# markomih/SplatFields

Hardware: AMD Instinct MI355X
Metric: splats*px rasterized/sec (fwd+bwd) (higher is better)
Workload: dtype f32

## Files before the change

### include/splatraster.h

```cpp
#ifndef SPLATRASTER_H
#define SPLATRASTER_H

#include <stddef.h>

#ifdef __cplusplus
extern "C" {
#endif

#define SR_VERSION 4
#define SR_TILE 16

typedef struct SrView {
    int image_height;
    int image_width;
    float tanfovx;
    float tanfovy;
    float scale_modifier;
    int sh_degree;
    int sh_coeffs;
    int prefiltered;
    int debug;
    const float* viewmatrix;
    const float* projmatrix;
    const float* campos;
// ... 218 lines not shown
    int count, rank, capacity;
} SrResFieldJob;
int sr_resfield_compose(int n_jobs, const SrResFieldJob* jobs, const long long* frame, void* hip_stream);
size_t sr_resfield_backward_workspace(int n_jobs, const SrResFieldJob* jobs);
int sr_resfield_backward(int n_jobs, const SrResFieldJob* jobs, const long long* frame, void* workspace, size_t workspace_bytes,
                         void* hip_stream);

size_t sr_triplane_backward_workspace(int n_points, int channels, int height, int width);
int sr_triplane_forward(int n_points, int channels, int height, int width, const float* planes, float* planes_texel_major,
                        const float* points, float* out, void* hip_stream);
int sr_triplane_backward(int n_points, int channels, int height, int width, const float* planes_texel_major, const float* points,
                         const float* dL_dout, float* dL_dplanes, float* dL_dpoints, void* workspace, void* hip_stream);

int sr_debug_layout(int n_splats, int height, int width, long long instances, size_t* out4);

int sr_debug_backward_stats(unsigned long long* out16, int reset);

int sr_debug_counters(long long* out4, int reset);

int sr_debug_snapshot(const SrView* view, const SrSplats* splats, const float* dL_dcolor, const float* dL_ddepth,
                      const float* dL_dalpha, int backward);

#define SR_PROFILE_STAGES 7
int sr_profile_enable(int on);
int sr_profile_collect(double* ms_sum, long long* launches);
const char* sr_profile_stage_name(int stage);

#ifdef __cplusplus
}
#endif
#endif
// ... 1 lines not shown
```

### splatfields_amd/csrc/api.hip

```cpp
#include <cstdint>
#include <cstdio>
#include <cstdlib>
#include <cstring>
#include <atomic>
#include <chrono>
#include <thread>
#include <mutex>
#include <string>
#include <vector>
#include "kernels.h"

namespace {

thread_local std::string g_last_error;
thread_local long long g_last_longest = -1;

int fail(const std::string& msg) { g_last_error = msg; return 1; }

int check_hip(hipError_t e, const char* what) {
    if (e == hipSuccess) return 0;
    return fail(std::string(what) + ": " + hipGetErrorString(e));
}

#define SR_TRY(expr) do { if (int rc_ = (expr)) return rc_; } while (0)
// ... 205 lines not shown
    sr::SplatsK k;
    k.N = s->count; k.means3D = s->means3D; k.opacities = s->opacities; k.scales = s->scales;
    k.rotations = s->rotations; k.cov3D = s->cov3D_precomp; k.shs = s->shs; k.colors = s->colors_precomp;
    k.raw = s->raw_params; k.shs_rest = s->shs_rest;
    return k;
}

long long covered_by_hint(long long hint) { return hint <= 2048 ? 2048 : hint <= 4096 ? 4096 : hint <= 8192 ? 8192 : -1; }

struct Call {
    hipStream_t st = nullptr;
    sr::ViewK v; sr::SplatsK s;
    sr::Geom g; sr::Binning b; sr::Image im;
    void carve(const void* geom, void* binning, long long capacity, const void* image) {
        sr::carve_geom(const_cast<void*>(geom), s.N, v.H, v.W, &g);
        if (binning) sr::carve_binning(binning, capacity, &b);
        if (image) sr::carve_image(const_cast<void*>(image), v.H, v.W, &im);
    }
};

int open_call(Call& c, const CallContext& ctx, void* hip_stream) {
    SR_TRY(validate(ctx.view, ctx.splats));
    g_call = ctx;
    c.st = static_cast<hipStream_t>(hip_stream);
    c.v = make_view(ctx.view);
    c.s = make_splats(ctx.splats);
    return 0;
}

bool capacity_in_range(long long r) { return r >= 0 && r < (1ll << 32); }

}

extern "C" {

int sr_version(void) { return SR_VERSION; }
const char* sr_last_error(void) { return g_last_error.c_str(); }

size_t sr_geom_bytes(int n, int h, int w) { return sr::carve_geom(nullptr, n, h, w, nullptr); }
size_t sr_binning_bytes(long long r, int, int) { return sr::carve_binning(nullptr, r, nullptr); }
size_t sr_image_bytes(int h, int w) { return sr::carve_image(nullptr, h, w, nullptr); }
size_t sr_backward_scratch_bytes(long long r) {
    const size_t n = (size_t)(r > 0 ? r : 1);
    return sr::align_up(n * sr::kSlotFloats * sizeof(float), 256);
}

}

namespace {

int launch_stage1(const SrView* view, const sr::ViewK& v, const sr::SplatsK& s, const sr::Geom& g, int* radii, uint32_t* host_out,
                  uint32_t host_seq, hipStream_t st) {
    { StageTimer t_(0, st); sr::launch_preprocess(v, s, g, radii, st); }
    SR_TRY(after_launch(view, st, "preprocess"));
    { StageTimer t_(1, st); sr::launch_count_tiles(v, s.N, g, st); sr::launch_scan_small(v, s.N, g, host_out, host_seq, st); }
// ... 540 lines not shown
                         const float* dL_dout, float* dL_dplanes, float* dL_dpoints, void* workspace, void* hip_stream) {
    if (n_points < 0 || !planes_texel_major || (n_points > 0 && (!points || !dL_dout)) || (dL_dplanes && !workspace))
        return fail("bad arguments to sr_triplane_backward");
    const int rc = sr::launch_triplane_backward(n_points, channels, height, width, planes_texel_major, points, dL_dout, dL_dplanes, dL_dpoints,
                                                workspace, static_cast<hipStream_t>(hip_stream));
    if (rc == 1) return fail("sr_triplane_backward: channels must be a multiple of 4 in 4..128, height * width <= 2^30, 12 n_points < 2^32");
    if (rc) return fail("sr_triplane_backward: clearing the tile counters failed");
    return check_hip(hipGetLastError(), "triplane_backward");
}

int sr_debug_layout(int n, int h, int w, long long instances, size_t* out4) {
    if (!out4 || n < 0 || h <= 0 || w <= 0 || instances < 0) return fail("bad arguments to sr_debug_layout");
    sr::Geom g; sr::Binning b;
    char* const origin = reinterpret_cast<char*>(4096);
    sr::carve_geom(origin, n, h, w, &g);
    sr::carve_binning(origin, instances, &b);
    out4[0] = (size_t)(reinterpret_cast<char*>(g.tile_start) - origin);
    out4[1] = (size_t)(reinterpret_cast<char*>(b.sorted_id) - origin);
    out4[2] = (size_t)(reinterpret_cast<char*>(g.total) - origin);
    out4[3] = (size_t)(reinterpret_cast<char*>(g.offsets) - origin);
    return 0;
}

int sr_debug_backward_stats(unsigned long long* out8, int reset) {
    if (!out8) return fail("null pointer in sr_debug_backward_stats");
    if (hipDeviceSynchronize() != hipSuccess) return fail("sr_debug_backward_stats: device synchronisation failed");
    return sr::backward_stats(out8, reset) ? fail("sr_debug_backward_stats: counter copy failed") : 0;
}

int sr_debug_snapshot(const SrView* view, const SrSplats* splats, const float* dL_dcolor, const float* dL_ddepth, const float* dL_dalpha,
                      int backward) {
    if (!view || !splats) return fail("null view/splats");
    g_call = CallContext{view, splats, backward ? "snapshot_bw.dump" : "snapshot_fw.dump", dL_dcolor, dL_ddepth, dL_dalpha};
    dump_snapshot(backward ? "render_backward (test hook)" : "preprocess (test hook)");
    return 0;
}

int sr_profile_enable(int on) { g_prof_on = on != 0; return 0; }

int sr_profile_collect(double* ms_sum, long long* launches) {
    std::lock_guard<std::mutex> lock(g_prof_mutex);
    std::vector<ProfRec> open;
// ... 17 lines not shown
```

### splatfields_amd/csrc/blend_bwd.hip

```cpp
#include "kernels.h"

namespace sr {

namespace {

constexpr int kBucket = 16;
constexpr int kBlkEntries = 32;
constexpr int kBlocks = 8;
#ifndef SR_BWD_CAP
#define SR_BWD_CAP 752
#endif
#ifndef SR_BWD_CAP_DEPTH
#define SR_BWD_CAP_DEPTH 624
#endif
template <bool HAS_D> struct SlotCap { static constexpr int kCap = HAS_D ? SR_BWD_CAP_DEPTH : SR_BWD_CAP; };
constexpr int kCapSlack = 16;
static_assert(SR_BWD_CAP >= 256 && SR_BWD_CAP_DEPTH >= 256, "one quad's entries of a chunk must always fit");
#ifndef SR_BWD_WAVES_PER_SIMD
#define SR_BWD_WAVES_PER_SIMD 4
#endif

typedef float f32x4 __attribute__((ext_vector_type(4)));

#ifdef SR_BWD_STATS
__device__ unsigned long long g_bwd_stats[16];
#define SR_STAT_ADD(i, x) atomicAdd(&g_bwd_stats[i], (unsigned long long)(x))
#define SR_PHASE(i) do { const long long now_ = clock64(); ph_[i] += now_ - t_; t_ = now_; } while (0)
#else
#define SR_STAT_ADD(i, x) do {} while (0)
#define SR_PHASE(i) do {} while (0)
#endif

constexpr int kShr1 = 0x111, kShr2 = 0x112, kShr4 = 0x114, kShr8 = 0x118;

template <int CTRL> __device__ __forceinline__ float dpp_f(float old, float src) {
    return __int_as_float(__builtin_amdgcn_update_dpp(__float_as_int(old), __float_as_int(src), CTRL, 0xf, 0xf, false));
}
template <int CTRL> __device__ __forceinline__ uint32_t dpp_u(uint32_t old, uint32_t src) {
    return (uint32_t)__builtin_amdgcn_update_dpp((int)old, (int)src, CTRL, 0xf, 0xf, false);
}
// ... 63 lines not shown
    const float4 r3 = rec[3];
    e.rect_xy = __float_as_uint(r3.x); e.rect_w = __float_as_uint(r3.y); e.first_rel = __float_as_uint(r3.z);
    e.inst = g.block_offsets[id >> 8];
    e.ef = make_float2(0.f, 0.f);
    e.qm = qms[pc];
    return e;
}
__device__ __forceinline__ void finish_entry(BwdEntry& e, uint32_t tx, uint32_t ty) {
    float E0, F0, ps;
    exponent_terms(e.c.x, e.c.y, e.r1, (float)(tx * kTile), (float)(ty * kTile), E0, F0, ps);
    e.ef = make_float2(E0, F0);
    e.r1.y = ps;
    e.inst += e.first_rel + (ty - (e.rect_xy >> 16)) * e.rect_w + (tx - (e.rect_xy & 0xffffu));
}

template <bool HAS_D> struct SlotFmt { static constexpr int kF = HAS_D ? 12 : 10; };

struct SlotIn { float E0, F0, p, ps, q, nlo, r, g, b, depth; int pos; };

template <bool HAS_D>
__device__ __forceinline__ void slot_put_record(float* sl, const BwdEntry& e) {
    if constexpr (HAS_D) {
        float4* d = reinterpret_cast<float4*>(sl);
        d[0] = make_float4(e.ef.x, e.ef.y, __int_as_float(e.pos), e.r1.x);
        d[1] = make_float4(e.r1.y, e.r1.z, e.r1.w, e.r2.x);
        d[2] = make_float4(e.r2.y, e.r2.z, e.r2.w, 0.f);
    } else {
        float2* d = reinterpret_cast<float2*>(sl);
        d[0] = make_float2(e.ef.x, e.ef.y);
        d[1] = make_float2(__int_as_float(e.pos), e.r1.x);
        d[2] = make_float2(e.r1.y, e.r1.z);
        d[3] = make_float2(e.r1.w, e.r2.x);
        d[4] = make_float2(e.r2.y, e.r2.z);
    }
}
template <bool HAS_D>
__device__ __forceinline__ SlotIn slot_get_record(const float* sl) {
    SlotIn r;
    if constexpr (HAS_D) {
        const float4* d = reinterpret_cast<const float4*>(sl);
        const float4 a = d[0], b = d[1], c = d[2];
        r.E0 = a.x; r.F0 = a.y; r.pos = __float_as_int(a.z); r.p = a.w;
        r.ps = b.x; r.q = b.y; r.nlo = b.z; r.r = b.w;
        r.g = c.x; r.b = c.y; r.depth = c.z;
    } else {
        const float2* d = reinterpret_cast<const float2*>(sl);
        const float2 a = d[0], b = d[1], c = d[2], e = d[3], f = d[4];
        r.E0 = a.x; r.F0 = a.y; r.pos = __float_as_int(b.x); r.p = b.y;
        r.ps = c.x; r.q = c.y; r.nlo = e.x; r.r = e.y;
        r.g = f.x; r.b = f.y; r.depth = 0.f;
    }
    return r;
}
__device__ __forceinline__ void slot_mask_invalid(SlotIn& r, bool valid) {
    r.nlo = valid ? r.nlo : __builtin_inff();
    r.r = valid ? r.r : 0.f; r.g = valid ? r.g : 0.f; r.b = valid ? r.b : 0.f; r.depth = valid ? r.depth : 0.f;
}
struct BucketSums { float w0, w1, w2; };
__device__ __forceinline__ void slot_put_sums(float* sl, int row, const BucketSums d) {
    const int o64 = row == 0 ? 0 : row == 1 ? 6 : row == 2 ? 4 : 8;
    *reinterpret_cast<float2*>(sl + o64) = row == 2 ? make_float2(d.w1, d.w2) : make_float2(d.w0, d.w1);
    if ((row & 1) == 0) sl[row == 0 ? 2 : 3] = row == 0 ? d.w2 : d.w0;
}
template <bool HAS_D>
__device__ __forceinline__ void slot_get_sums(const float* sl, float4& a, float4& b, float2& c) {
    if constexpr (HAS_D) {
        const float4* d = reinterpret_cast<const float4*>(sl);
        const float4 x = d[0], y = d[1], z = d[2];
        a = make_float4(x.x, x.w, y.z, z.x); b = make_float4(x.y, y.x, y.w, z.y); c = make_float2(x.z, y.y);
    } else {
        const float2* d = reinterpret_cast<const float2*>(sl);
        const float2 x0 = d[0], x1 = d[1], x2 = d[2], x3 = d[3], x4 = d[4];
        a = make_float4(x0.x, x1.y, x3.x, x4.x); b = make_float4(x0.y, x2.x, x3.y, x4.y); c = make_float2(x1.x, x2.y);
    }
}

__constant__ float kColumn[3][16] = {
    {0.f, 1.f, 2.f, 3.f, 4.f, 5.f, 6.f, 7.f, 8.f, 9.f, 10.f, 11.f, 12.f, 13.f, 14.f, 15.f},
    {-7.5f, -6.5f, -5.5f, -4.5f, -3.5f, -2.5f, -1.5f, -0.5f, 0.5f, 1.5f, 2.5f, 3.5f, 4.5f, 5.5f, 6.5f, 7.5f},
    {56.25f, 42.25f, 30.25f, 20.25f, 12.25f, 6.25f, 2.25f, 0.25f, 0.25f, 2.25f, 6.25f, 12.25f, 20.25f, 30.25f, 42.25f, 56.25f}};

struct QuadCtx {
    float gR[4], gG[4], gB[4], gD[4], gA[4];
    int last[4];
    float Y;
    float Xa[4], Xc[4], Xc2[4];
};

#define SR_DPP_MUL4(ctrl) \
// ... 69 lines not shown
    const float Yc = c.Y - 7.5f;
    const float mY = Yc * a0, mXY = Yc * a1, mYY = Yc * mY;
    BucketSums r;
    r.w0 = swap16_sum(swap32_sum(a0, a1), swap32_sum(mY, a2));
    r.w1 = swap16_sum(swap32_sum(mXY, mYY), swap32_sum(br, bg));
    const float zz = swap32_sum(bb, bd);
    r.w2 = swap16_sum(zz, zz);
    (void)lane;
    return r;
}

template <bool HAS_D>
__global__ void __launch_bounds__(kBlock, SR_BWD_WAVES_PER_SIMD)
k_render_backward_quads(const ViewK v, const Geom g, const Binning b, const Image im, const float* __restrict__ dL_dcolor,
                       const float* __restrict__ dL_ddepth, const float* __restrict__ dL_dalpha, float* __restrict__ slots) {
    constexpr int kF = SlotFmt<HAS_D>::kF;
    constexpr int kCap = SlotCap<HAS_D>::kCap;
    __shared__ __attribute__((aligned(16))) float s_slot[(kCap + kCapSlack) * kF];
    __shared__ float4 s_pixA[256];
    __shared__ float4 s_pixB[256];
    __shared__ uint32_t s_mask[2][16][kBlocks];
    __shared__ uint16_t s_bb[2][16][kBlocks];
    __shared__ uint32_t s_qlen[2][16], s_qbase[2][16];
    __shared__ uint32_t s_ticket[2];

    const int tile = (int)g.tile_order[blockIdx.x];
    const int tx = tile % v.gx, ty = tile / v.gx;
    const int wave = wave_id(), lane = lane_id();
    const uint32_t start = g.tile_start[tile];
    const float tx0f = (float)(tx * kTile), ty0f = (float)(ty * kTile);
#ifdef SR_BWD_STATS
    long long ph_[8] = {0, 0, 0, 0, 0, 0, 0, 0}, t_ = clock64();
#endif
// ... 1 lines not shown
    const int tid = (int)threadIdx.x;
    const uint32_t* ids = b.sorted_id + start;

    uint32_t qlast[16];
    {
        const uint32_t* ql = g.tile_qlast + 16 * (size_t)tile;
#pragma unroll
        for (int q = 0; q < 16; ++q) qlast[q] = ql[q];
    }
    uint32_t bmax_u = 0u, qlast_min = 0xffffffffu;
#pragma unroll
    for (int q = 0; q < 16; ++q) { bmax_u = max(bmax_u, qlast[q]); qlast_min = min(qlast_min, qlast[q]); }
    const int bmax = __builtin_amdgcn_readfirstlane((int)bmax_u);
    qlast_min = (uint32_t)__builtin_amdgcn_readfirstlane((int)qlast_min);

    constexpr int kChunk = kBlocks * kBlkEntries;
    static_assert(kChunk == kBlock, "one list entry per thread");
    if (bmax == 0) return;
    int hi = bmax;
    const uint32_t* qms = b.qmask + start;
    const uint32_t id_first = ids[max(hi - 1 - tid, 0)];
    uint32_t id_next = ids[max(hi - kChunk - 1 - tid, 0)];
    BwdEntry cur = load_entry(g, id_first, qms, hi - 1 - tid);

    {
        const int lx = threadIdx.x & 15, ly = threadIdx.x >> 4;
        const int px = tx * kTile + lx, py = ty * kTile + ly;
        const bool inside = px < v.W && py < v.H;
        const size_t hw = (size_t)v.H * v.W, pix = (size_t)py * v.W + px;
        uint32_t my_last = 0;
        float T_final = 0.f, gR = 0.f, gG = 0.f, gB = 0.f, gD = 0.f, gA = 0.f;
        if (inside) {
            my_last = im.n_contrib[pix];
            T_final = im.final_T[pix];
            gR = dL_dcolor[pix]; gG = dL_dcolor[hw + pix]; gB = dL_dcolor[2 * hw + pix];
            if (HAS_D) gD = dL_ddepth[pix];
            if (dL_dalpha) gA = dL_dalpha[pix];
        }
// ... 2 lines not shown
        s_pixB[threadIdx.x] = make_float4(gA, __uint_as_float(my_last), T_final, T_final * bg_dot);
        if (threadIdx.x < 2) s_ticket[threadIdx.x] = 0u;
    }

    const int k = lane >> 4, nl = lane & 15;
    const uint32_t lt_mask = (1u << (lane & 31)) - 1u;
    const int myblk = (int)threadIdx.x >> 5;

    float4* slot4 = reinterpret_cast<float4*>(slots);
    const float4 zero4 = make_float4(0.f, 0.f, 0.f, 0.f);

    int par = 0;
    SR_PHASE(0);

    while (hi > 0) {
        uint32_t qm = 0u;
        if (cur.pos >= 0) {
            qm = cur.qm & 0xffffu;
            if ((uint32_t)cur.pos >= qlast_min) {
#pragma unroll
                for (int q = 0; q < 16; ++q) if ((uint32_t)cur.pos >= qlast[q]) qm &= ~(1u << q);
            }
        }
        {
            uint32_t mlo = 0u, mhi = 0u;
#pragma unroll
            for (int q = 0; q < 16; ++q) {
                const uint64_t bal = __builtin_amdgcn_ballot_w64(((qm >> q) & 1u) != 0u);
                asm("s_nop 3\n\tv_writelane_b32 %0, %2, %4\n\tv_writelane_b32 %1, %3, %4"
                    : "+v"(mlo), "+v"(mhi) : "s"((uint32_t)bal), "s"((uint32_t)(bal >> 32)), "n"(q));
// ... 22 lines not shown
                for (int qq = 0; qq < 16; ++qq) {
                    const uint32_t pq = (uint32_t)__builtin_amdgcn_readlane((int)len, qq);
                    if (run + pq > (uint32_t)kCap) { pass_starts |= 1u << qq; run = 0u; }
                    my_base = q == qq ? run : my_base;
                    run += pq;
                }
            }
            if (lane < 16) {
                s_qlen[par][q] = len; s_qbase[par][q] = my_base;
#pragma unroll
                for (int blk = 0; blk < kBlocks; ++blk) s_bb[par][q][blk] = (uint16_t)(my_base + first_of[blk]);
            }
            if (threadIdx.x == 0) s_ticket[par ^ 1] = 0u;
#ifdef SR_BWD_STATS
            { const uint32_t pairs = row_allsum_u32(len);
              if (threadIdx.x == 0) { SR_STAT_ADD(0, min(hi, kChunk)); SR_STAT_ADD(1, pairs); SR_STAT_ADD(5, 1); } }
#endif
            __builtin_amdgcn_fence(__ATOMIC_RELEASE, "wavefront");
            __builtin_amdgcn_wave_barrier();
            __builtin_amdgcn_fence(__ATOMIC_ACQUIRE, "wavefront");
        }
        float4 s0 = zero4, s1 = zero4;
        float2 s2 = make_float2(0.f, 0.f);
        pass_starts = (uint32_t)__builtin_amdgcn_readfirstlane((int)pass_starts) | 0x10000u;
        uint32_t last_pmask = 0u;
        auto combine = [&](uint32_t pmask) {
            if (cur.pos >= 0) {
                uint32_t m = qm & pmask;
                while (m) {
                    const int q = __builtin_ctz(m);
                    m &= m - 1u;
                    const uint32_t slot = (uint32_t)s_bb[par][q][myblk] + (uint32_t)__popc(s_mask[par][q][myblk] & lt_mask);
                    float4 a, cc; float2 d;
                    slot_get_sums<HAS_D>(s_slot + kF * slot, a, cc, d);
                    s0.x += a.x; s0.y += a.y; s0.z += a.z; s0.w += a.w;
                    s1.x += cc.x; s1.y += cc.y; s1.z += cc.z; s1.w += cc.w;
                    s2.x += d.x; if (HAS_D) s2.y += d.y;
                }
            }
        };
#pragma unroll 1
        for (int q_lo = 0; q_lo < 16;) {
            const int q_hi = __builtin_ctz(pass_starts & ~((2u << q_lo) - 1u));
            const uint32_t pmask = ((1u << q_hi) - 1u) & ~((1u << q_lo) - 1u);
            if (q_lo == 0) finish_entry(cur, (uint32_t)tx, (uint32_t)ty);
            {
                uint32_t m = qm & pmask;
                while (m) {
                    const int q = __builtin_ctz(m);
                    m &= m - 1u;
                    const uint32_t slot = (uint32_t)s_bb[par][q][myblk] + (uint32_t)__popc(s_mask[par][q][myblk] & lt_mask);
                    slot_put_record<HAS_D>(s_slot + kF * slot, cur);
                }
            }
            if (threadIdx.x == 0) s_ticket[par] = (uint32_t)q_lo;
            SR_PHASE(3);
            lds_barrier();
            SR_PHASE(4);
            uint32_t ticket = 0u;
            if (lane == 0) ticket = atomicAdd(&s_ticket[par], 1u);
#pragma unroll 1
            for (;;) {
                const int q = __builtin_amdgcn_readfirstlane((int)ticket);
                if (q >= q_hi) break;
                if (lane == 0) ticket = atomicAdd(&s_ticket[par], 1u);
                const int qy = q >> 2, qx = q & 3;
                const int len = __builtin_amdgcn_readfirstlane((int)s_qlen[par][q]);
// ... 2 lines not shown
                const int prow = (4 * qy + k) * 16 + 4 * qx;
                QuadCtx c;
                float ST[4], SB[4];
                c.Y = (float)(4 * qy + k);
#pragma unroll
                for (int t = 0; t < 4; ++t) {
                    c.Xa[t] = kColumn[0][4 * qx + t]; c.Xc[t] = kColumn[1][4 * qx + t]; c.Xc2[t] = kColumn[2][4 * qx + t];
                }
#pragma unroll
                for (int t = 0; t < 4; ++t) {
                    const float4 a = s_pixA[prow + t], cb = s_pixB[prow + t];
                    c.gR[t] = a.x; c.gG[t] = a.y; c.gB[t] = a.z; c.gD[t] = a.w;
                    c.gA[t] = cb.x; c.last[t] = __float_as_int(cb.y); ST[t] = cb.z; SB[t] = cb.w;
                }
                const int last_bucket = ((len - 1) >> 4) << 4;
                auto slot_of = [&](int i, bool up) { return s_slot + kF * (base + min(i, last_bucket) + (up ? nl : 15 - nl)); };
                int i0 = 0;
#pragma unroll 1
                for (; i0 + kBucket < len; i0 += 2 * kBucket) {
                    float* sa = slot_of(i0, true);
                    float* sb = slot_of(i0 + kBucket, false);
                    const SlotIn ea = slot_get_record<HAS_D>(sa);
                    SlotIn eb = slot_get_record<HAS_D>(sb);
                    const bool vb = i0 + kBucket + (15 - nl) < len;
                    slot_mask_invalid(eb, vb);
#ifdef SR_BWD_STATS
                    if (lane == 0) { SR_STAT_ADD(2, 2); SR_STAT_ADD(3, 16 * (kBucket + min(kBucket, len - i0 - kBucket))); }
#endif
                    const BucketSums Da = replay_bucket<true, HAS_D>(c, ea, ST, SB, lane);
                    const BucketSums Db = replay_bucket<false, HAS_D>(c, eb, ST, SB, lane);
                    slot_put_sums(sa, k, Da);
                    if (vb) slot_put_sums(sb, k, Db);
                }
                const bool tail = i0 < len;
                if (tail) {
                    float* sa = slot_of(i0, true);
                    SlotIn ea = slot_get_record<HAS_D>(sa);
                    const bool va = i0 + nl < len;
                    slot_mask_invalid(ea, va);
#ifdef SR_BWD_STATS
                    if (lane == 0) { SR_STAT_ADD(2, 1); SR_STAT_ADD(3, 16 * min(kBucket, len - i0)); }
#endif
                    const BucketSums Da = replay_bucket<true, HAS_D>(c, ea, ST, SB, lane);
                    if (va) slot_put_sums(sa, k, Da);
                }
                if (nl == (tail ? 15 : 0)) {
#pragma unroll
                    for (int t = 0; t < 4; ++t) {
                        float* st = reinterpret_cast<float*>(&s_pixB[prow + t]);
                        st[2] = ST[t]; st[3] = SB[t];
                    }
                }
            }
            SR_PHASE(5);
            lds_barrier();
            SR_PHASE(6);
            if (q_hi == 16) { last_pmask = pmask; break; }
            combine(pmask);
            lds_barrier();
            q_lo = q_hi;
        }
        combine(last_pmask);
        hi -= kChunk;
        par ^= 1;
        const float2 centre = cur.c;
        const size_t inst = cur.inst;
        const bool has_entry = cur.pos >= 0;
        if (has_entry) {
            const float ox = centre.x - (tx0f + 7.5f), oy = centre.y - (ty0f + 7.5f);
            const float M0 = s0.x, MX = s0.y, MY = s0.z, MXX = s0.w, MXY = s1.x, MYY = s1.y;
            const float Sx = ox * M0 - MX, Sy = oy * M0 - MY;
            const float Sxx = fmaf(ox, Sx - MX, MXX);
            const float Syy = fmaf(oy, Sy - MY, MYY);
            const float Sxy = fmaf(ox, Sy, MXY) - oy * MX;
            slot4[inst * kSlotF4] = make_float4(M0, Sx, Sy, Sxx);
            slot4[inst * kSlotF4 + 1] = make_float4(Sxy, Syy, s1.z, s1.w);
            slot4[inst * kSlotF4 + 2] = make_float4(s2.x, s2.y, 0.f, 0.f);
            b.reached[inst] = 1;
        }
        if (hi > 0) {
            cur = load_entry(g, id_next, qms, hi - 1 - tid);
            id_next = ids[max(hi - kChunk - 1 - tid, 0)];
        }
        SR_PHASE(7);
    }
#ifdef SR_BWD_STATS
    if (lane == 0) for (int i = 0; i < 8; ++i) SR_STAT_ADD(8 + i, ph_[i]);
#endif
}

int backward_stats(unsigned long long* out8, int reset) {
#ifdef SR_BWD_STATS
    if (hipMemcpyFromSymbol(out8, HIP_SYMBOL(g_bwd_stats), 16 * sizeof(unsigned long long)) != hipSuccess) return 1;
    if (reset) {
        unsigned long long z[16] = {0, 0, 0, 0, 0, 0, 0, 0, 0, 0, 0, 0, 0, 0, 0, 0};
        if (hipMemcpyToSymbol(HIP_SYMBOL(g_bwd_stats), z, sizeof(z)) != hipSuccess) return 1;
    }
    return 0;
#else
    for (int i = 0; i < 16; ++i) out8[i] = 0ull;
    (void)reset;
    return 0;
#endif
}

void launch_render_backward_quads(const ViewK& v, const Geom& g, const Binning& b, const Image& im,
                                 const float* dL_dcolor, const float* dL_ddepth, const float* dL_dalpha,
                                 float* slots, hipStream_t st) {
    const int tiles = v.gx * v.gy;
    if (tiles <= 0) return;
    if (dL_ddepth) hipLaunchKernelGGL(k_render_backward_quads<true>, dim3(tiles), dim3(kBlock), 0, st, v, g, b, im, dL_dcolor, dL_ddepth, dL_dalpha, slots);
    else hipLaunchKernelGGL(k_render_backward_quads<false>, dim3(tiles), dim3(kBlock), 0, st, v, g, b, im, dL_dcolor, dL_ddepth, dL_dalpha, slots);
}

}
// ... 1 lines not shown
```

### splatfields_amd/csrc/common.h

```cpp
#pragma once
#include <hip/hip_runtime.h>
#include <stdint.h>
#include "../../include/splatraster.h"

namespace sr {

constexpr int kTile = SR_TILE;
constexpr int kSub = 8;
constexpr float kNearCullZ = 0.2f;
constexpr float kDilation = 0.3f;
constexpr float kClampFov = 1.3f;
constexpr float kAlphaMax = 0.99f;
constexpr float kAlphaMin = 1.0f / 255.0f;
constexpr float kTStop = 0.0001f;
constexpr float kWEps = 0.0000001f;

constexpr float SH_C0 = 0.28209479177387814f;
constexpr float SH_C1 = 0.4886025119029199f;
constexpr float SH_C2_0 = 1.0925484305920792f, SH_C2_1 = -1.0925484305920792f, SH_C2_2 = 0.31539156525252005f,
                SH_C2_3 = -1.0925484305920792f, SH_C2_4 = 0.5462742152960396f;
constexpr float SH_C3_0 = -0.5900435899266435f, SH_C3_1 = 2.890611442640554f, SH_C3_2 = -0.4570457994644658f,
                SH_C3_3 = 0.3731763325901154f, SH_C3_4 = -0.4570457994644658f, SH_C3_5 = 1.445305721320277f,
                SH_C3_6 = -0.5900435899266435f;

// ... 36 lines not shown
    c.chunks = (c.n_sub + c.sub_per_chunk - 1) / c.sub_per_chunk;
    c.slices = 1;
    if (c.sub_per_chunk == 1) { c.slices = kMaxChunks / c.chunks; if (c.slices > 8) c.slices = 8; if (c.slices < 1) c.slices = 1; }
    c.chunks *= c.slices;
    c.segments = (c.chunks + kSegRows - 1) / kSegRows;
    c.tiles_padded = (tiles + 63) / 64 * 64;
    return c;
}

struct Binning {
    uint64_t* ent;
    uint64_t* keys;
    uint64_t* keys_tmp;
    uint32_t* sorted_id;
    uint32_t* qmask;
    uint8_t* reached;
    uint32_t capacity;
    uint32_t sorted_up_to;
};

struct Image {
    float* final_T;
    uint32_t* n_contrib;
};

__host__ __device__ inline size_t align_up(size_t x, size_t a) { return (x + a - 1) / a * a; }

struct Carver {
    char* base; size_t off;
    template <typename T> __host__ T* take(size_t n) {
// ... 21 lines not shown
    t.block_sums = c.take<uint32_t>(nb); t.block_offsets = c.take<uint32_t>(nb);
    t.tile_count = c.take<uint32_t>(tiles); t.tile_start = c.take<uint32_t>(tiles + 1);
    t.tile_cursor = c.take<uint32_t>(tiles); t.tile_order = c.take<uint32_t>(tiles); t.total = c.take<uint32_t>(8);
    t.tile_qlast = c.take<uint32_t>(16 * tiles);
    t.cnt = t.segtot = t.segbase = nullptr;
    if (tiles <= (size_t)kMaxMatrixTiles) {
        const Chunking ch = make_chunking(N, (int)tiles);
        t.cnt = c.take<uint32_t>((size_t)ch.chunks * ch.tiles_padded);
        t.segtot = c.take<uint32_t>((size_t)ch.segments * ch.tiles_padded);
        t.segbase = c.take<uint32_t>((size_t)ch.segments * ch.tiles_padded);
    }
    if (g) *g = t;
    return align_up(c.off, 256);
}

inline size_t carve_binning(void* base, long long R, Binning* b) {
    Carver c{static_cast<char*>(base), 0};
    const size_t r = (size_t)(R > 0 ? R : 1);
    Binning t;
    t.ent = c.take<uint64_t>(r);
    t.keys = c.take<uint64_t>(r);
    t.keys_tmp = c.take<uint64_t>(r);
    t.sorted_id = c.take<uint32_t>(r);
    t.qmask = c.take<uint32_t>(r);
    t.reached = c.take<uint8_t>(r);
    t.capacity = (uint32_t)(R > 0 ? R : 0);
    t.sorted_up_to = 0xffffffffu;
    if (b) *b = t;
    return align_up(c.off, 256);
}

inline size_t carve_image(void* base, int H, int W, Image* im) {
    Carver c{static_cast<char*>(base), 0};
    const size_t px = (size_t)H * W;
    Image t;
    t.final_T = c.take<float>(px); t.n_contrib = c.take<uint32_t>(px);
    if (im) *im = t;
    return align_up(c.off, 256);
}

// ... 189 lines not shown
```

### splatfields_amd/csrc/kernels.h

```cpp
#pragma once
#include "common.h"

namespace sr {

struct SplatsK {
    int N;
    const float* means3D; const float* opacities; const float* scales; const float* rotations;
    const float* cov3D; const float* shs; const float* colors;
    int raw;
    const float* shs_rest;
};

struct GradsK {
    float* means3D; float* means2D; float* opacity; float* scales; float* rotations; float* cov3D;
    float* shs; float* colors; float* shs_rest;
};

void launch_preprocess(const ViewK& v, const SplatsK& s, const Geom& g, int* radii, hipStream_t st);
void launch_mark_visible(int N, const float* means3D, const float* viewmatrix, unsigned char* present, hipStream_t st);
void launch_densification_stats(int N, const float* dL_dmeans2D, const int* radii, float* grad_accum, float* denom, float* max_radii2D,
                                hipStream_t st);
void launch_preprocess_backward(const ViewK& v, const SplatsK& s, const Geom& g, const int* radii,
                                const float* slots, const uint8_t* reached, const GradsK& gr, int first, int count, bool small_footprint,
                                hipStream_t st);
inline bool use_count_matrix(const ViewK& v) { return v.gx * v.gy <= kMaxMatrixTiles; }
void launch_count_tiles(const ViewK& v, int N, const Geom& g, hipStream_t st);
void launch_scan_small(const ViewK& v, int N, const Geom& g, uint32_t* host_out, uint32_t host_seq, hipStream_t st);
void launch_emit(const ViewK& v, int N, const Geom& g, const Binning& b, hipStream_t st);
void launch_sort_tiles(const ViewK& v, const Geom& g, const Binning& b, long long max_len, long long expected_len, hipStream_t st);
void launch_render_forward(const ViewK& v, const Geom& g, const Binning& b, const Image& im,
                           float* out_color, float* out_depth, float* out_alpha, hipStream_t st);
void launch_render_backward(const ViewK& v, const Geom& g, const Binning& b, const Image& im,
                            const float* dL_dcolor, const float* dL_ddepth, const float* dL_dalpha,
                            float* slots, hipStream_t st);
void launch_render_backward_quads(const ViewK& v, const Geom& g, const Binning& b, const Image& im,
                                 const float* dL_dcolor, const float* dL_ddepth, const float* dL_dalpha,
                                 float* slots, hipStream_t st);

int backward_stats(unsigned long long* out8, int reset);

struct DensifyArgs { float grad_threshold, min_opacity, extent, percent_dense, max_screen_size; };
size_t densify_workspace_bytes(int n);
void launch_densify_plan(int n, const float* log_scales, int scale_cols, const float* opacity_logit, const float* grad_accum,
                         const float* denom, const float* max_radii2D, const DensifyArgs& a, void* workspace, int32_t* dest,
                         uint32_t** totals_out, hipStream_t st);
void launch_densify_gather(int n, int row, const float* src, float* dst, const int32_t* dest, int mode, const float* log_scales,
                           int scale_cols, const float* rotations, const float* unit, hipStream_t st);

size_t mlp_weight_grad_workspace(int n_points, int n_jobs, const SrMlpGradJob* jobs);
int launch_mlp_weight_grad(int n_points, int n_jobs, const SrMlpGradJob* jobs, void* workspace, size_t workspace_bytes, hipStream_t st);
int launch_mlp_pack(int n_jobs, const SrMlpPackJob* jobs, hipStream_t st);
int launch_mlp_chain(int n_points, int hidden_tiles, int n_ops, const SrMlpOp* ops, float slope, hipStream_t st);

int launch_mlp_input_forward(int N, int L, int F, int TL, int row, const float* xyz, const float* feat, const float* time, float* x0, hipStream_t st);
// ... 61 lines not shown
```

### splatfields_amd/csrc/render.hip

```cpp
#include "kernels.h"
#define SR_QM_DEVICE 1
#include "quadmask.h"

namespace sr {

constexpr int kBwdBatch = 128;

__device__ __forceinline__ void wave_lds_fence() {
    __builtin_amdgcn_fence(__ATOMIC_RELEASE, "wavefront");
    __builtin_amdgcn_wave_barrier();
    __builtin_amdgcn_fence(__ATOMIC_ACQUIRE, "wavefront");
}

typedef unsigned int uint2v __attribute__((ext_vector_type(2)));

__device__ __forceinline__ float mask_select(uint64_t mask, float a, float b) {
    float r;
    asm("v_cndmask_b32_e64 %0, %1, %2, %3" : "=v"(r) : "v"(b), "v"(a), "s"(mask));
    return r;
}
__device__ __forceinline__ uint32_t mask_select(uint64_t mask, uint32_t a, uint32_t b) {
    uint32_t r;
    asm("v_cndmask_b32_e64 %0, %1, %2, %3" : "=v"(r) : "v"(b), "v"(a), "s"(mask));
    return r;
// ... 65 lines not shown
    if (start == end) {
        goto done;
    }
    {
    auto stages = [&](uint32_t k) { return kStagers == 4 || (uint32_t)(wave >> 1) == (k & 1u); };
    const int slot = kStagers == 4 ? (int)threadIdx.x : (int)(threadIdx.x & 127u);
    const int wslot = kStagers == 4 ? wave : (wave & 1);
    const uint32_t l0 = lds_address(&s_r0[0][wslot * kWave]), l1 = lds_address(&s_r1[0][wslot * kWave]), l2 = lds_address(&s_r2[0][wslot * kWave]);
    constexpr uint32_t kCopyStride = kB * sizeof(float4);
    auto request = [&](int buf, uint32_t id) {
        const float4* rec = g.rec + 4 * (size_t)id;
        lds_copy16_async(rec, l0 + buf * kCopyStride);
        lds_copy16_async(rec + 1, l1 + buf * kCopyStride);
        lds_copy16_async(rec + 2, l2 + buf * kCopyStride);
    };
    auto publish_mask = [&](int buf, uint32_t i) {
        uint32_t qm = 0u;
        if (i < end) {
            const float4 r0 = s_r0[buf][slot], r1 = s_r1[buf][slot];
            qm = sr_quad_mask(r0.x, r0.y, r0.z, r1.x, r1.y, r1.z, tx0f, ty0f);
            b.qmask[i] = qm;
            float E0, F0, ps;
            exponent_terms(r0.x, r0.y, r1, tx0f, ty0f, E0, F0, ps);
            *reinterpret_cast<float2*>(&s_r0[buf][slot]) = make_float2(E0, F0);
            s_r1[buf][slot].y = ps;
        }
        s_qm[buf][slot] = (uint16_t)qm;
    };
    const uint32_t lastpos = end - 1u;
    const uint32_t i0 = start + (uint32_t)slot;
    const uint32_t k_first = kStagers == 4 ? 1u : ((wave >> 1) == 1 ? 1u : 2u);
    uint32_t id_nxt = b.sorted_id[min(i0 + k_first * kB, lastpos)];
    if (stages(0u)) {
        const uint32_t id0 = b.sorted_id[min(i0, lastpos)];
        request(0, id0);
        lds_copy_wait();
        publish_mask(0, i0);
    }
    asm volatile("" :: "v"(id_nxt));
    lds_barrier();

    uint32_t k = 0;
// ... 266 lines not shown
```

Measured before the change: 1303000 billion.

## Fit backward chunks to LDS slot capacity using per-group pair counts

The forward blend kernel now records, for each 64-entry group of a tile's sorted list, the number of quad-pixel pairs. The backward kernel uses these counts to choose variable-size chunks that fill the LDS slot budget, instead of always taking a fixed chunk of 256 entries. With depth enabled, slot records shrink from 12 floats to 10 floats plus a 16-bit relative position, and the depth slot cap rises from 624 to 720. This aims to cut the number of backward passes and overflow handling, at the cost of an extra global buffer, extra DPP reductions in the forward pass, and more control logic in the backward loop.

```diff
diff --git a/include/splatraster.h b/include/splatraster.h
--- a/include/splatraster.h
+++ b/include/splatraster.h
@@ -256,7 +256,7 @@
 
 int sr_debug_layout(int n_splats, int height, int width, long long instances, size_t* out4);
 
-int sr_debug_backward_stats(unsigned long long* out16, int reset);
+int sr_debug_backward_stats(unsigned long long* out24, int reset);
 
 int sr_debug_counters(long long* out4, int reset);
 
diff --git a/splatfields_amd/csrc/api.hip b/splatfields_amd/csrc/api.hip
--- a/splatfields_amd/csrc/api.hip
+++ b/splatfields_amd/csrc/api.hip
@@ -243,7 +243,7 @@
     sr::Geom g; sr::Binning b; sr::Image im;
     void carve(const void* geom, void* binning, long long capacity, const void* image) {
         sr::carve_geom(const_cast<void*>(geom), s.N, v.H, v.W, &g);
-        if (binning) sr::carve_binning(binning, capacity, &b);
+        if (binning) sr::carve_binning(binning, capacity, v.H, v.W, &b);
         if (image) sr::carve_image(const_cast<void*>(image), v.H, v.W, &im);
     }
 };
@@ -267,7 +267,7 @@
 const char* sr_last_error(void) { return g_last_error.c_str(); }
 
 size_t sr_geom_bytes(int n, int h, int w) { return sr::carve_geom(nullptr, n, h, w, nullptr); }
-size_t sr_binning_bytes(long long r, int, int) { return sr::carve_binning(nullptr, r, nullptr); }
+size_t sr_binning_bytes(long long r, int h, int w) { return sr::carve_binning(nullptr, r, h, w, nullptr); }
 size_t sr_image_bytes(int h, int w) { return sr::carve_image(nullptr, h, w, nullptr); }
 size_t sr_backward_scratch_bytes(long long r) {
     const size_t n = (size_t)(r > 0 ? r : 1);
@@ -838,7 +838,7 @@
     sr::Geom g; sr::Binning b;
     char* const origin = reinterpret_cast<char*>(4096);
     sr::carve_geom(origin, n, h, w, &g);
-    sr::carve_binning(origin, instances, &b);
+    sr::carve_binning(origin, instances, h, w, &b);
     out4[0] = (size_t)(reinterpret_cast<char*>(g.tile_start) - origin);
     out4[1] = (size_t)(reinterpret_cast<char*>(b.sorted_id) - origin);
     out4[2] = (size_t)(reinterpret_cast<char*>(g.total) - origin);
@@ -846,10 +846,10 @@
     return 0;
 }
 
-int sr_debug_backward_stats(unsigned long long* out8, int reset) {
-    if (!out8) return fail("null pointer in sr_debug_backward_stats");
+int sr_debug_backward_stats(unsigned long long* out24, int reset) {
+    if (!out24) return fail("null pointer in sr_debug_backward_stats");
     if (hipDeviceSynchronize() != hipSuccess) return fail("sr_debug_backward_stats: device synchronisation failed");
-    return sr::backward_stats(out8, reset) ? fail("sr_debug_backward_stats: counter copy failed") : 0;
+    return sr::backward_stats(out24, reset) ? fail("sr_debug_backward_stats: counter copy failed") : 0;
 }
 
 int sr_debug_snapshot(const SrView* view, const SrSplats* splats, const float* dL_dcolor, const float* dL_ddepth, const float* dL_dalpha,
diff --git a/splatfields_amd/csrc/blend_bwd.hip b/splatfields_amd/csrc/blend_bwd.hip
--- a/splatfields_amd/csrc/blend_bwd.hip
+++ b/splatfields_amd/csrc/blend_bwd.hip
@@ -7,11 +7,26 @@
 constexpr int kBucket = 16;
 constexpr int kBlkEntries = 32;
 constexpr int kBlocks = 8;
+#ifndef SR_BWD_CHUNK_BLOCKS
+#define SR_BWD_CHUNK_BLOCKS 8
+#endif
+#ifndef SR_BWD_MIN_FIT_GROUPS
+#define SR_BWD_MIN_FIT_GROUPS 2
+#endif
+constexpr int kChunkBlocks = SR_BWD_CHUNK_BLOCKS;
+static_assert(kChunkBlocks >= 2 && kChunkBlocks <= kBlocks && kChunkBlocks % 2 == 0, "a chunk holds whole groups, at most one entry per thread");
+constexpr int kGroup = 64;
+constexpr int kMinFit = SR_BWD_MIN_FIT_GROUPS * kGroup;
+#ifdef SR_BWD_FIXED_CHUNKS
+constexpr bool kFitChunks = false;
+#else
+constexpr bool kFitChunks = true;
+#endif
 #ifndef SR_BWD_CAP
 #define SR_BWD_CAP 752
 #endif
 #ifndef SR_BWD_CAP_DEPTH
-#define SR_BWD_CAP_DEPTH 624
+#define SR_BWD_CAP_DEPTH 720
 #endif
 template <bool HAS_D> struct SlotCap { static constexpr int kCap = HAS_D ? SR_BWD_CAP_DEPTH : SR_BWD_CAP; };
 constexpr int kCapSlack = 16;
@@ -23,7 +38,7 @@
 typedef float f32x4 __attribute__((ext_vector_type(4)));
 
 #ifdef SR_BWD_STATS
-__device__ unsigned long long g_bwd_stats[16];
+__device__ unsigned long long g_bwd_stats[24];
 #define SR_STAT_ADD(i, x) atomicAdd(&g_bwd_stats[i], (unsigned long long)(x))
 #define SR_PHASE(i) do { const long long now_ = clock64(); ph_[i] += now_ - t_; t_ = now_; } while (0)
 #else
@@ -117,42 +132,30 @@
     e.inst += e.first_rel + (ty - (e.rect_xy >> 16)) * e.rect_w + (tx - (e.rect_xy & 0xffffu));
 }
 
-template <bool HAS_D> struct SlotFmt { static constexpr int kF = HAS_D ? 12 : 10; };
+constexpr int kF = 10;
 
 struct SlotIn { float E0, F0, p, ps, q, nlo, r, g, b, depth; int pos; };
 
 template <bool HAS_D>
-__device__ __forceinline__ void slot_put_record(float* sl, const BwdEntry& e) {
-    if constexpr (HAS_D) {
-        float4* d = reinterpret_cast<float4*>(sl);
-        d[0] = make_float4(e.ef.x, e.ef.y, __int_as_float(e.pos), e.r1.x);
-        d[1] = make_float4(e.r1.y, e.r1.z, e.r1.w, e.r2.x);
-        d[2] = make_float4(e.r2.y, e.r2.z, e.r2.w, 0.f);
-    } else {
-        float2* d = reinterpret_cast<float2*>(sl);
-        d[0] = make_float2(e.ef.x, e.ef.y);
-        d[1] = make_float2(__int_as_float(e.pos), e.r1.x);
-        d[2] = make_float2(e.r1.y, e.r1.z);
-        d[3] = make_float2(e.r1.w, e.r2.x);
-        d[4] = make_float2(e.r2.y, e.r2.z);
-    }
+__device__ __forceinline__ void slot_put_record(float* sl, uint16_t* rel, const BwdEntry& e, int first_pos) {
+    float2* d = reinterpret_cast<float2*>(sl);
+    d[0] = make_float2(e.ef.x, e.ef.y);
+    d[1] = make_float2(HAS_D ? e.r2.w : __int_as_float(e.pos), e.r1.x);
+    d[2] = make_float2(e.r1.y, e.r1.z);
+    d[3] = make_float2(e.r1.w, e.r2.x);
+    d[4] = make_float2(e.r2.y, e.r2.z);
+    if (HAS_D) *rel = (uint16_t)(first_pos - e.pos);
 }
 template <bool HAS_D>
-__device__ __forceinline__ SlotIn slot_get_record(const float* sl) {
+__device__ __forceinline__ SlotIn slot_get_record(const float* sl, const uint16_t* rel, int first_pos) {
     SlotIn r;
-    if constexpr (HAS_D) {
-        const float4* d = reinterpret_cast<const float4*>(sl);
-        const float4 a = d[0], b = d[1], c = d[2];
-        r.E0 = a.x; r.F0 = a.y; r.pos = __float_as_int(a.z); r.p = a.w;
-        r.ps = b.x; r.q = b.y; r.nlo = b.z; r.r = b.w;
-        r.g = c.x; r.b = c.y; r.depth = c.z;
-    } else {
-        const float2* d = reinterpret_cast<const float2*>(sl);
-        const float2 a = d[0], b = d[1], c = d[2], e = d[3], f = d[4];
-        r.E0 = a.x; r.F0 = a.y; r.pos = __float_as_int(b.x); r.p = b.y;
-        r.ps = c.x; r.q = c.y; r.nlo = e.x; r.r = e.y;
-        r.g = f.x; r.b = f.y; r.depth = 0.f;
-    }
+    const float2* d = reinterpret_cast<const float2*>(sl);
+    const float2 a = d[0], b = d[1], c = d[2], e = d[3], f = d[4];
+    r.E0 = a.x; r.F0 = a.y; r.p = b.y;
+    r.ps = c.x; r.q = c.y; r.nlo = e.x; r.r = e.y;
+    r.g = f.x; r.b = f.y;
+    if (HAS_D) { r.depth = b.x; r.pos = first_pos - (int)*rel; }
+    else { r.depth = 0.f; r.pos = __float_as_int(b.x); }
     return r;
 }
 __device__ __forceinline__ void slot_mask_invalid(SlotIn& r, bool valid) {
@@ -165,17 +168,10 @@
     *reinterpret_cast<float2*>(sl + o64) = row == 2 ? make_float2(d.w1, d.w2) : make_float2(d.w0, d.w1);
     if ((row & 1) == 0) sl[row == 0 ? 2 : 3] = row == 0 ? d.w2 : d.w0;
 }
-template <bool HAS_D>
 __device__ __forceinline__ void slot_get_sums(const float* sl, float4& a, float4& b, float2& c) {
-    if constexpr (HAS_D) {
-        const float4* d = reinterpret_cast<const float4*>(sl);
-        const float4 x = d[0], y = d[1], z = d[2];
-        a = make_float4(x.x, x.w, y.z, z.x); b = make_float4(x.y, y.x, y.w, z.y); c = make_float2(x.z, y.y);
-    } else {
-        const float2* d = reinterpret_cast<const float2*>(sl);
-        const float2 x0 = d[0], x1 = d[1], x2 = d[2], x3 = d[3], x4 = d[4];
-        a = make_float4(x0.x, x1.y, x3.x, x4.x); b = make_float4(x0.y, x2.x, x3.y, x4.y); c = make_float2(x1.x, x2.y);
-    }
+    const float2* d = reinterpret_cast<const float2*>(sl);
+    const float2 x0 = d[0], x1 = d[1], x2 = d[2], x3 = d[3], x4 = d[4];
+    a = make_float4(x0.x, x1.y, x3.x, x4.x); b = make_float4(x0.y, x2.x, x3.y, x4.y); c = make_float2(x1.x, x2.y);
 }
 
 __constant__ float kColumn[3][16] = {
@@ -275,9 +271,9 @@
 __global__ void __launch_bounds__(kBlock, SR_BWD_WAVES_PER_SIMD)
 k_render_backward_quads(const ViewK v, const Geom g, const Binning b, const Image im, const float* __restrict__ dL_dcolor,
                        const float* __restrict__ dL_ddepth, const float* __restrict__ dL_dalpha, float* __restrict__ slots) {
-    constexpr int kF = SlotFmt<HAS_D>::kF;
     constexpr int kCap = SlotCap<HAS_D>::kCap;
     __shared__ __attribute__((aligned(16))) float s_slot[(kCap + kCapSlack) * kF];
+    __shared__ uint16_t s_rel[HAS_D ? kCap + kCapSlack : 1];
     __shared__ float4 s_pixA[256];
     __shared__ float4 s_pixB[256];
     __shared__ uint32_t s_mask[2][16][kBlocks];
@@ -309,14 +305,38 @@
     const int bmax = __builtin_amdgcn_readfirstlane((int)bmax_u);
     qlast_min = (uint32_t)__builtin_amdgcn_readfirstlane((int)qlast_min);
 
-    constexpr int kChunk = kBlocks * kBlkEntries;
-    static_assert(kChunk == kBlock, "one list entry per thread");
+    constexpr int kChunk = kChunkBlocks * kBlkEntries;
+    static_assert(kChunk <= kBlock, "at most one list entry per thread");
     if (bmax == 0) return;
     int hi = bmax;
     const uint32_t* qms = b.qmask + start;
+    const uint32_t* gpairs = b.group_pairs + group_pairs_base(start, tile);
+    auto load_groups = [&](int top_group) { return kFitChunks ? gpairs[max(top_group - (lane & 7), 0)] : 0u; };
+    int gref = (hi - 1) >> 6;
+    uint32_t gv = load_groups(gref);
+    auto cut = [&](int top) -> int {
+        if (!kFitChunks) return max(top - kChunk, 0);
+        const int lo_full = (max(top - kChunk, 0) + kGroup - 1) & ~(kGroup - 1);
+        const int g = (top - 1) >> 6;
+        int lo = g << 6;
+        uint32_t sum = (uint32_t)__builtin_amdgcn_readlane((int)gv, gref - g);
+        bool open = true;
+#pragma unroll
+        for (int j = 1; j < kChunkBlocks / 2; ++j) {
+            const uint32_t x = (uint32_t)__builtin_amdgcn_readlane((int)gv, min(gref - g + j, 7));
+            open = open && lo - kGroup >= lo_full && sum <= (uint32_t)kCap && x <= (uint32_t)kCap - sum;
+            lo = open ? lo - kGroup : lo;
+            sum = open ? sum + x : sum;
+        }
+        if (lo > lo_full && (top - lo < kMinFit || sum > (uint32_t)kCap)) lo = lo_full;
+        return __builtin_amdgcn_readfirstlane(lo);
+    };
     const uint32_t id_first = ids[max(hi - 1 - tid, 0)];
-    uint32_t id_next = ids[max(hi - kChunk - 1 - tid, 0)];
     BwdEntry cur = load_entry(g, id_first, qms, hi - 1 - tid);
+    int lo = cut(hi);
+    int lo2 = 0;
+    if (cur.pos < lo) cur.pos = -1;
+    uint32_t id_next = ids[max(lo - 1 - tid, 0)];
 
     {
         const int lx = threadIdx.x & 15, ly = threadIdx.x >> 4;
@@ -349,6 +369,7 @@
     SR_PHASE(0);
 
     while (hi > 0) {
+        lo2 = lo > 0 ? cut(lo) : 0;
         uint32_t qm = 0u;
         if (cur.pos >= 0) {
             qm = cur.qm & 0xffffu;
@@ -401,7 +422,12 @@
             if (threadIdx.x == 0) s_ticket[par ^ 1] = 0u;
 #ifdef SR_BWD_STATS
             { const uint32_t pairs = row_allsum_u32(len);
-              if (threadIdx.x == 0) { SR_STAT_ADD(0, min(hi, kChunk)); SR_STAT_ADD(1, pairs); SR_STAT_ADD(5, 1); } }
+              const int passes = __popc(pass_starts & 0xffffu);
+              if (threadIdx.x == 0) {
+                  SR_STAT_ADD(0, hi - lo); SR_STAT_ADD(1, pairs); SR_STAT_ADD(5, 1);
+                  SR_STAT_ADD(16, passes); SR_STAT_ADD(passes >= 3 ? 19 : 16 + passes, 1);
+                  if (hi - lo == kChunk) { SR_STAT_ADD(20, 1); SR_STAT_ADD(21, pairs); SR_STAT_ADD(22, pairs > (uint32_t)kCap ? 1 : 0); }
+              } }
 #endif
             __builtin_amdgcn_fence(__ATOMIC_RELEASE, "wavefront");
             __builtin_amdgcn_wave_barrier();
@@ -419,7 +445,7 @@
                     m &= m - 1u;
                     const uint32_t slot = (uint32_t)s_bb[par][q][myblk] + (uint32_t)__popc(s_mask[par][q][myblk] & lt_mask);
                     float4 a, cc; float2 d;
-                    slot_get_sums<HAS_D>(s_slot + kF * slot, a, cc, d);
+                    slot_get_sums(s_slot + kF * slot, a, cc, d);
                     s0.x += a.x; s0.y += a.y; s0.z += a.z; s0.w += a.w;
                     s1.x += cc.x; s1.y += cc.y; s1.z += cc.z; s1.w += cc.w;
                     s2.x += d.x; if (HAS_D) s2.y += d.y;
@@ -437,7 +463,7 @@
                     const int q = __builtin_ctz(m);
                     m &= m - 1u;
                     const uint32_t slot = (uint32_t)s_bb[par][q][myblk] + (uint32_t)__popc(s_mask[par][q][myblk] & lt_mask);
-                    slot_put_record<HAS_D>(s_slot + kF * slot, cur);
+                    slot_put_record<HAS_D>(s_slot + kF * slot, s_rel + (HAS_D ? slot : 0u), cur, hi - 1);
                 }
             }
             if (threadIdx.x == 0) s_ticket[par] = (uint32_t)q_lo;
@@ -470,14 +496,16 @@
                     c.gA[t] = cb.x; c.last[t] = __float_as_int(cb.y); ST[t] = cb.z; SB[t] = cb.w;
                 }
                 const int last_bucket = ((len - 1) >> 4) << 4;
-                auto slot_of = [&](int i, bool up) { return s_slot + kF * (base + min(i, last_bucket) + (up ? nl : 15 - nl)); };
+                auto slot_of = [&](int i, bool up) { return base + min(i, last_bucket) + (up ? nl : 15 - nl); };
+                auto record_of = [&](int slot) { return slot_get_record<HAS_D>(s_slot + kF * slot, s_rel + (HAS_D ? slot : 0), hi - 1); };
                 int i0 = 0;
 #pragma unroll 1
                 for (; i0 + kBucket < len; i0 += 2 * kBucket) {
-                    float* sa = slot_of(i0, true);
-                    float* sb = slot_of(i0 + kBucket, false);
-                    const SlotIn ea = slot_get_record<HAS_D>(sa);
-                    SlotIn eb = slot_get_record<HAS_D>(sb);
+                    const int ia = slot_of(i0, true), ib = slot_of(i0 + kBucket, false);
+                    float* sa = s_slot + kF * ia;
+                    float* sb = s_slot + kF * ib;
+                    const SlotIn ea = record_of(ia);
+                    SlotIn eb = record_of(ib);
                     const bool vb = i0 + kBucket + (15 - nl) < len;
                     slot_mask_invalid(eb, vb);
 #ifdef SR_BWD_STATS
@@ -490,8 +518,9 @@
                 }
                 const bool tail = i0 < len;
                 if (tail) {
-                    float* sa = slot_of(i0, true);
-                    SlotIn ea = slot_get_record<HAS_D>(sa);
+                    const int ia = slot_of(i0, true);
+                    float* sa = s_slot + kF * ia;
+                    SlotIn ea = record_of(ia);
                     const bool va = i0 + nl < len;
                     slot_mask_invalid(ea, va);
 #ifdef SR_BWD_STATS
@@ -517,7 +546,7 @@
             q_lo = q_hi;
         }
         combine(last_pmask);
-        hi -= kChunk;
+        hi = lo; lo = lo2;
         par ^= 1;
         const float2 centre = cur.c;
         const size_t inst = cur.inst;
@@ -535,8 +564,10 @@
             b.reached[inst] = 1;
         }
         if (hi > 0) {
-            cur = load_entry(g, id_next, qms, hi - 1 - tid);
-            id_next = ids[max(hi - kChunk - 1 - tid, 0)];
+            const int p = hi - 1 - tid;
+            cur = load_entry(g, id_next, qms, p >= lo ? p : -1);
+            id_next = ids[max(lo - 1 - tid, 0)];
+            if (lo > 0) { gref = (lo - 1) >> 6; gv = load_groups(gref); }
         }
         SR_PHASE(7);
     }
@@ -545,16 +576,16 @@
 #endif
 }
 
-int backward_stats(unsigned long long* out8, int reset) {
-#ifdef SR_BWD_STATS
-    if (hipMemcpyFromSymbol(out8, HIP_SYMBOL(g_bwd_stats), 16 * sizeof(unsigned long long)) != hipSuccess) return 1;
+int backward_stats(unsigned long long* out24, int reset) {
+#ifdef SR_BWD_STATS
+    if (hipMemcpyFromSymbol(out24, HIP_SYMBOL(g_bwd_stats), 24 * sizeof(unsigned long long)) != hipSuccess) return 1;
     if (reset) {
-        unsigned long long z[16] = {0, 0, 0, 0, 0, 0, 0, 0, 0, 0, 0, 0, 0, 0, 0, 0};
+        unsigned long long z[24] = {};
         if (hipMemcpyToSymbol(HIP_SYMBOL(g_bwd_stats), z, sizeof(z)) != hipSuccess) return 1;
     }
     return 0;
 #else
-    for (int i = 0; i < 16; ++i) out8[i] = 0ull;
+    for (int i = 0; i < 24; ++i) out24[i] = 0ull;
     (void)reset;
     return 0;
 #endif
diff --git a/splatfields_amd/csrc/common.h b/splatfields_amd/csrc/common.h
--- a/splatfields_amd/csrc/common.h
+++ b/splatfields_amd/csrc/common.h
@@ -74,6 +74,7 @@
     uint64_t* keys_tmp;
     uint32_t* sorted_id;
     uint32_t* qmask;
+    uint32_t* group_pairs;
     uint8_t* reached;
     uint32_t capacity;
     uint32_t sorted_up_to;
@@ -125,7 +126,9 @@
     return align_up(c.off, 256);
 }
 
-inline size_t carve_binning(void* base, long long R, Binning* b) {
+__host__ __device__ inline size_t group_pairs_base(uint32_t tile_start, int tile) { return (size_t)(tile_start >> 6) + (size_t)tile; }
+
+inline size_t carve_binning(void* base, long long R, int H, int W, Binning* b) {
     Carver c{static_cast<char*>(base), 0};
     const size_t r = (size_t)(R > 0 ? R : 1);
     Binning t;
@@ -135,6 +138,7 @@
     t.sorted_id = c.take<uint32_t>(r);
     t.qmask = c.take<uint32_t>(r);
     t.reached = c.take<uint8_t>(r);
+    t.group_pairs = c.take<uint32_t>(r / 64 + (size_t)tiles_x(W) * tiles_y(H) + 1);
     t.capacity = (uint32_t)(R > 0 ? R : 0);
     t.sorted_up_to = 0xffffffffu;
     if (b) *b = t;
diff --git a/splatfields_amd/csrc/kernels.h b/splatfields_amd/csrc/kernels.h
--- a/splatfields_amd/csrc/kernels.h
+++ b/splatfields_amd/csrc/kernels.h
@@ -37,7 +37,7 @@
                                  const float* dL_dcolor, const float* dL_ddepth, const float* dL_dalpha,
                                  float* slots, hipStream_t st);
 
-int backward_stats(unsigned long long* out8, int reset);
+int backward_stats(unsigned long long* out24, int reset);
 
 struct DensifyArgs { float grad_threshold, min_opacity, extent, percent_dense, max_screen_size; };
 size_t densify_workspace_bytes(int n);
diff --git a/splatfields_amd/csrc/render.hip b/splatfields_amd/csrc/render.hip
--- a/splatfields_amd/csrc/render.hip
+++ b/splatfields_amd/csrc/render.hip
@@ -103,6 +103,7 @@
         lds_copy16_async(rec + 1, l1 + buf * kCopyStride);
         lds_copy16_async(rec + 2, l2 + buf * kCopyStride);
     };
+    uint32_t* const group_pairs = b.group_pairs + group_pairs_base(start, tile);
     auto publish_mask = [&](int buf, uint32_t i) {
         uint32_t qm = 0u;
         if (i < end) {
@@ -115,6 +116,14 @@
             s_r1[buf][slot].y = ps;
         }
         s_qm[buf][slot] = (uint16_t)qm;
+        uint32_t np = (uint32_t)__popc(qm & 0xffffu);
+        np += (uint32_t)__builtin_amdgcn_update_dpp(0, (int)np, 0xB1, 0xf, 0xf, false);
+        np += (uint32_t)__builtin_amdgcn_update_dpp(0, (int)np, 0x4E, 0xf, 0xf, false);
+        np += (uint32_t)__builtin_amdgcn_update_dpp(0, (int)np, 0x124, 0xf, 0xf, false);
+        np += (uint32_t)__builtin_amdgcn_update_dpp(0, (int)np, 0x128, 0xf, 0xf, false);
+        const uint32_t group_np = (uint32_t)(__builtin_amdgcn_readlane((int)np, 0) + __builtin_amdgcn_readlane((int)np, 16) +
+                                             __builtin_amdgcn_readlane((int)np, 32) + __builtin_amdgcn_readlane((int)np, 48));
+        if (lane == 0 && i < end) group_pairs[(i - start) >> 6] = group_np;
     };
     const uint32_t lastpos = end - 1u;
     const uint32_t i0 = start + (uint32_t)slot;
```

Result: slower. 1255000 billion (-3.7%).
